# apple/ml-pgdvs

Measured on AMD Instinct MI355X. Metric: novel-view frames/s at 1080p x 24 src frames; achieved HBM GB/s vs gfx950 peak, higher is better.
Workload: dtype f32

## Files before the change

### ml-pgdvs_amd/csrc/knn_grid.hip

```cpp
#include <stdlib.h>

#include "common.h"
#include "fused.h"
#include "wave.h"

namespace pgdvs {

constexpr int kGridMaxCells = 1 << 24;
constexpr int kRingCap = 24;
constexpr int kRingCapAfterTpq = 3;
constexpr float kTargetPerCellDefault = 18.0f;

struct GridParams {
  float mn[3];
  float h, inv_h;
  int G[3];
  int ncells;
  int n;
  float sample_dist;
  int sample_dists;
};

__global__ void __launch_bounds__(256)
grid_bbox_kernel(const float *__restrict__ pts, const int32_t *__restrict__ count,
// ... 541 lines not shown
      *reinterpret_cast<int4 *>(out + idx) = q;
    } else if (idx <= n) {
      out[idx] = q.x;
      if (idx + 1 <= n) out[idx + 1] = q.y;
      if (idx + 2 <= n) out[idx + 2] = q.z;
    }
  }
  __syncthreads();
  }
}

__device__ __forceinline__ int wave_cell_take(int32_t *__restrict__ remaining, int c) {
  const int lane = threadIdx.x & 63;
  RunInfo r = wave_runs(c);
  int base = 0;
  if (r.is_leader && c >= 0) base = atomicSub(&remaining[c], r.length) - r.length;
  base = __shfl(base, r.leader, 64);
  return base + (lane - r.leader);
}

__global__ void __launch_bounds__(256)
grid_fill_kernel(const float *__restrict__ pts, const GridParams *__restrict__ gp,
                 const int32_t *__restrict__ cell_of, const int32_t *__restrict__ cell_start,
                 int32_t *__restrict__ cell_count, float4 *__restrict__ sorted,
                 const int32_t *__restrict__ gate) {
  if (gate && *gate == 0) return;
  const int n = gp->n;
  const int n_round = (n + 63) / 64 * 64;
  for (int i = blockIdx.x * blockDim.x + threadIdx.x; i < n_round; i += gridDim.x * blockDim.x) {
    const int c = i < n ? cell_of[i] : -1;
    const int slot = wave_cell_take(cell_count, c);
    if (i < n)
      sorted[cell_start[c] + slot] = make_float4(pts[(size_t)i * 3], pts[(size_t)i * 3 + 1], pts[(size_t)i * 3 + 2],
                                                 __int_as_float(i));
  }
}

struct BestList {
  float best;
  float mx;
};

__device__ __forceinline__ float readlane_f(float v, int l) {
  return __int_as_float(__builtin_amdgcn_readlane(__float_as_int(v), l));
}

__device__ __forceinline__ float wave_shift_up1_zero(float v) {
  int r = __builtin_amdgcn_update_dpp(0, __float_as_int(v), 0x138, 0xf, 0xf, true);
  return __int_as_float(r);
}

__device__ __forceinline__ void best_insert_batch(BestList &b, float d, bool valid, int KK, int lane) {
  (void)lane;
  unsigned long long mask = __ballot(valid && d < b.mx);
  if (!mask) return;
  while (mask) {
    int l = __builtin_ctzll(mask);
    mask &= mask - 1;
    float v = readlane_f(d, l);
    float up = wave_shift_up1_zero(b.best);
    b.best = __builtin_amdgcn_fmed3f(b.best, up, v);
  }
  b.mx = readlane_f(b.best, KK - 1);
}

template <int J>
__device__ __forceinline__ float lane_xor(float v, int lane) {
  const int iv = __float_as_int(v);
  if (J == 1) return __int_as_float(__builtin_amdgcn_update_dpp(iv, iv, 0xB1, 0xf, 0xf, false));
  if (J == 2) return __int_as_float(__builtin_amdgcn_update_dpp(iv, iv, 0x4E, 0xf, 0xf, false));
  if (J == 4) {
    int t = __builtin_amdgcn_update_dpp(iv, iv, 0x104, 0xf, 0x5, false);
    t = __builtin_amdgcn_update_dpp(t, iv, 0x114, 0xf, 0xa, false);
    return __int_as_float(t);
  }
  if (J == 8) return __int_as_float(__builtin_amdgcn_update_dpp(iv, iv, 0x128, 0xf, 0xf, false));
  if (J == 16) {
    auto r = __builtin_amdgcn_permlane16_swap(iv, iv, false, false);
    return __int_as_float((lane & 16) ? r[0] : r[1]);
  }
  auto r = __builtin_amdgcn_permlane32_swap(iv, iv, false, false);
  return __int_as_float((lane & 32) ? r[0] : r[1]);
}

template <int K, int J>
__device__ __forceinline__ float sort_step(float v, int lane) {
  const float o = lane_xor<J>(v, lane);
  const bool up = (lane & K) == 0;
  const bool lower = (lane & J) == 0;
  const float mn = fminf(v, o), mx = fmaxf(v, o);
  return (up == lower) ? mn : mx;
}

__device__ __forceinline__ float wave_sort_asc(float v, int lane) {
  v = sort_step<2, 1>(v, lane);
  v = sort_step<4, 2>(v, lane);
  v = sort_step<4, 1>(v, lane);
  v = sort_step<8, 4>(v, lane);
  v = sort_step<8, 2>(v, lane);
  v = sort_step<8, 1>(v, lane);
  v = sort_step<16, 8>(v, lane);
  v = sort_step<16, 4>(v, lane);
  v = sort_step<16, 2>(v, lane);
  v = sort_step<16, 1>(v, lane);
  v = sort_step<32, 16>(v, lane);
  v = sort_step<32, 8>(v, lane);
  v = sort_step<32, 4>(v, lane);
  v = sort_step<32, 2>(v, lane);
  v = sort_step<32, 1>(v, lane);
  v = sort_step<64, 32>(v, lane);
  v = sort_step<64, 16>(v, lane);
  v = sort_step<64, 8>(v, lane);
  v = sort_step<64, 4>(v, lane);
  v = sort_step<64, 2>(v, lane);
  v = sort_step<64, 1>(v, lane);
  return v;
}

__device__ __forceinline__ float dist2(float qx, float qy, float qz, float4 p) {
  float dx = qx - p.x, dy = qy - p.y, dz = qz - p.z;
  float d = dx * dx;
  d = d + dy * dy;
  d = d + dz * dz;
  return d;
}

__device__ __forceinline__ void scan_range(BestList &b, bool &first, const float4 *__restrict__ sorted,
                                           int start, int end, float qx, float qy, float qz, int KK,
                                           int lane, float bound = __builtin_inff()) {
  for (int j0 = start; j0 < end; j0 += 256) {
    float d[4];
    bool v[4];
#pragma unroll
    for (int u = 0; u < 4; ++u) {
      int j = j0 + u * 64 + lane;
      v[u] = j < end;
      float4 p = v[u] ? sorted[j] : make_float4(0.f, 0.f, 0.f, 0.f);
      d[u] = dist2(qx, qy, qz, p);
      v[u] = v[u] && d[u] <= bound;
    }
#pragma unroll
    for (int u = 0; u < 4; ++u) {
      if (j0 + u * 64 >= end) break;
      if (first) {
        b.best = wave_sort_asc(v[u] ? d[u] : __builtin_inff(), lane);
        b.mx = readlane_f(b.best, KK - 1);
        first = false;
      } else {
        best_insert_batch(b, d[u], v[u], KK, lane);
      }
    }
  }
}

struct QuerySrc {
  const float *qpts;
  const int32_t *qcount;
  int first_col;
  const int32_t *list;
  const int32_t *list_count;
  const float4 *qsorted;
};

__device__ __forceinline__ int query_count(const QuerySrc &qs, int n_points) {
  return qs.list ? *qs.list_count : (qs.qpts ? *qs.qcount : n_points);
}

__device__ __forceinline__ float4 load_query(const QuerySrc &qs, const float4 *__restrict__ sorted, int q) {
  if (qs.qpts == nullptr) return (qs.qsorted ? qs.qsorted : sorted)[q];
  return make_float4(qs.qpts[(size_t)q * 3], qs.qpts[(size_t)q * 3 + 1], qs.qpts[(size_t)q * 3 + 2],
                     __int_as_float(q));
}

__device__ __forceinline__ void knn_finish(float best, int KK, int first_col, int n, int lane, int orig,
                                           float *__restrict__ avg_out) {
  float s = (lane >= first_col && lane < KK && lane < n) ? best : 0.0f;
  s = wave_sum_down(s);
  if (lane == 0) avg_out[orig] = s / (float)(KK - first_col);
}

__device__ __forceinline__ float box_axis_dist2(float q, float mn, float h, int c0, int c1, int G) {
  float lo = c0 <= 0 ? -__builtin_inff() : mn + (float)c0 * h - 0.02f * h;
  float hi = c1 >= G - 1 ? __builtin_inff() : mn + (float)(c1 + 1) * h + 0.02f * h;
  float d = fmaxf(fmaxf(lo - q, q - hi), 0.0f);
  return d * d;
}

__device__ __forceinline__ void
grid_query_body(const GridParams *__restrict__ gp, const float4 *__restrict__ sorted,
                const CellIndex cell_start, int KK, QuerySrc qs, float *__restrict__ avg_out,
                int32_t *__restrict__ stats, int ring_cap, int32_t *__restrict__ fb_count,
                int32_t *__restrict__ fb_list, float *__restrict__ fb_bound) {
  const GridParams g = *gp;
  const int lane = threadIdx.x & 63;
  const int wave = __builtin_amdgcn_readfirstlane((int)(threadIdx.x >> 6));
  const int nq = query_count(qs, g.n);
  for (int qi = blockIdx.x * 4 + wave; qi < nq; qi += gridDim.x * 4) {
  const int q = qs.list ? qs.list[qi] : qi;
  const float4 qp = load_query(qs, sorted, q);
  const float qx = qp.x, qy = qp.y, qz = qp.z;
  const int orig = __float_as_int(qp.w);
  if (qs.qpts && !(isfinite(qx) && isfinite(qy) && isfinite(qz))) {
    if (lane == 0) avg_out[orig] = __builtin_nanf("");
    continue;
  }
  const int cx = cell_coord(qx, g.mn[0], g.inv_h, g.G[0]);
  const int cy = cell_coord(qy, g.mn[1], g.inv_h, g.G[1]);
  const int cz = cell_coord(qz, g.mn[2], g.inv_h, g.G[2]);
  BestList b;
  b.best = __builtin_inff();
  b.mx = __builtin_inff();
  bool first = true;
  bool done = false;
  int rings = 0;
  for (int r = 1; r <= ring_cap && !done; ++r) {
    rings = r;
    const int side = 2 * r + 1;
    const int nrows = side * side;
    for (int base = 0; base < nrows; base += 64) {
      int row_id = base + lane;
      if (r == 1) row_id = row_id < 9 ? (int)((0x862071534ull >> (row_id * 4)) & 15) : row_id;
      int s0 = 0, e0 = 0, s1 = 0, e1 = 0;
      float bd0 = 0.0f, bd1 = 0.0f;
      if (row_id < nrows) {
        int rz = (int)(((float)row_id + 0.5f) / (float)side);
        int dz = rz - r, dy = row_id - rz * side - r;
        int z = cz + dz, y = cy + dy;
        if (z >= 0 && z < g.G[2] && y >= 0 && y < g.G[1]) {
          int row = (z * g.G[1] + y) * g.G[0];
          float byz = box_axis_dist2(qy, g.mn[1], g.h, y, y, g.G[1]) + box_axis_dist2(qz, g.mn[2], g.h, z, z, g.G[2]);
          bool outer = r == 1 || dz == -r || dz == r || dy == -r || dy == r;
          if (outer) {
            int x0 = cx - r < 0 ? 0 : cx - r;
            int x1 = cx + r >= g.G[0] ? g.G[0] - 1 : cx + r;
            s0 = cell_start.at(row + x0);
            e0 = cell_start.at(row + x1 + 1);
            bd0 = byz + box_axis_dist2(qx, g.mn[0], g.h, x0, x1, g.G[0]);
          } else {
            if (cx - r >= 0) {
              s0 = cell_start.at(row + cx - r);
              e0 = cell_start.at(row + cx - r + 1);
              bd0 = byz + box_axis_dist2(qx, g.mn[0], g.h, cx - r, cx - r, g.G[0]);
            }
            if (cx + r < g.G[0]) {
              s1 = cell_start.at(row + cx + r);
              e1 = cell_start.at(row + cx + r + 1);
              bd1 = byz + box_axis_dist2(qx, g.mn[0], g.h, cx + r, cx + r, g.G[0]);
            }
          }
        }
      }
      unsigned long long m0 = __ballot(e0 > s0);
      while (m0) {
        int l = __builtin_ctzll(m0);
        m0 &= m0 - 1;
        if (readlane_f(bd0, l) >= b.mx) continue;
        scan_range(b, first, sorted, __builtin_amdgcn_readlane(s0, l), __builtin_amdgcn_readlane(e0, l), qx,
                   qy, qz, KK, lane);
      }
      unsigned long long m1 = __ballot(e1 > s1);
      while (m1) {
        int l = __builtin_ctzll(m1);
        m1 &= m1 - 1;
        if (readlane_f(bd1, l) >= b.mx) continue;
        scan_range(b, first, sorted, __builtin_amdgcn_readlane(s1, l), __builtin_amdgcn_readlane(e1, l), qx,
                   qy, qz, KK, lane);
      }
    }
    float db = __builtin_inff();
    bool open = false;
    const int c[3] = {cx, cy, cz};
    const float qv[3] = {qx, qy, qz};
#pragma unroll
    for (int a = 0; a < 3; ++a) {
      if (c[a] - r > 0) {
        open = true;
        db = fminf(db, qv[a] - (g.mn[a] + (float)(c[a] - r) * g.h));
      }
      if (c[a] + r < g.G[a] - 1) {
        open = true;
        db = fminf(db, (g.mn[a] + (float)(c[a] + r + 1) * g.h) - qv[a]);
      }
    }
    if (!open) {
      done = true;
    } else {
      float safe = db - 0.02f * g.h;
      if (safe > 0.0f && b.mx <= safe * safe) done = true;
    }
  }
  if (stats && lane == 0) atomicAdd(&stats[done ? (rings < 15 ? rings : 14) : 15], 1);
  if (!done) {
    if (lane == 0) {
      int slot = atomicAdd(fb_count, 1);
      fb_list[slot] = q;
      fb_bound[slot] = b.mx;
    }
    continue;
  }
  knn_finish(b.best, KK, qs.first_col, g.n, lane, orig, avg_out);
  }
}

constexpr int kTpqQueue = 8;
constexpr float kTpqRetryScale = 4.0f;

template <int KK>
__device__ __forceinline__ void tpq_insert(float (&a)[KK], float c) {
#pragma unroll
  for (int i = KK - 1; i > 0; --i) a[i] = __builtin_amdgcn_fmed3f(a[i - 1], a[i], c);
  asm("v_min_f32 %0, %1, %2" : "=v"(a[0]) : "v"(a[0]), "v"(c));
}

template <int KK>
__global__ void __launch_bounds__(256, 4)
grid_query_tpq_kernel(const GridParams *__restrict__ gp, const float4 *__restrict__ sorted,
                      const CellIndex cell_start, int first_col, float *__restrict__ avg_out,
                      int32_t *__restrict__ open_count, int32_t *__restrict__ open_list, float thr_mult) {
  __shared__ int2 s_run[9][256];
  __shared__ float s_bd[9][256];
  __shared__ float s_thr[256];
  __shared__ float s_safe[256];
  __shared__ unsigned long long s_order[256];
  const GridParams g = *gp;
  const int n = g.n;
  const int tid = threadIdx.x;
  for (int q0 = blockIdx.x * 256; q0 < n; q0 += gridDim.x * 256) {
  const int q = q0 + tid;
  const bool live = q < n;
  const float4 qp = sorted[live ? q : n - 1];
  const float qx = qp.x, qy = qp.y, qz = qp.z;
  float t0;
  {
  int ncand = 0;
  const int cx = cell_coord(qx, g.mn[0], g.inv_h, g.G[0]);
  const int cy = cell_coord(qy, g.mn[1], g.inv_h, g.G[1]);
  const int cz = cell_coord(qz, g.mn[2], g.inv_h, g.G[2]);
  const int x0 = cx - 1 < 0 ? 0 : cx - 1;
  const int x1 = cx + 1 >= g.G[0] ? g.G[0] - 1 : cx + 1;
#pragma unroll
  for (int k = 0; k < 9; ++k) {
    const int z = cz + k / 3 - 1, y = cy + k % 3 - 1;
    if (live && z >= 0 && z < g.G[2] && y >= 0 && y < g.G[1]) {
      const int row = (z * g.G[1] + y) * g.G[0];
      ncand += cell_start.at(row + x1 + 1) - cell_start.at(row + x0);
    }
  }
  t0 = (KK >= 17 && ncand >= KK) ? (KK >= 40 ? thr_mult : 6.0f) * (float)KK * g.h * g.h / (float)ncand : __builtin_inff();
  {
    float db = __builtin_inff();
    bool open = false;
    const int c[3] = {cx, cy, cz};
    const float qv[3] = {qx, qy, qz};
#pragma unroll
    for (int ax = 0; ax < 3; ++ax) {
      if (c[ax] - 1 > 0) {
        open = true;
        db = fminf(db, qv[ax] - (g.mn[ax] + (float)(c[ax] - 1) * g.h));
      }
      if (c[ax] + 1 < g.G[ax] - 1) {
        open = true;
        db = fminf(db, (g.mn[ax] + (float)(c[ax] + 2) * g.h) - qv[ax]);
      }
    }
    const float safe = db - 0.02f * g.h;
    s_safe[tid] = !open ? __builtin_inff() : (safe > 0.0f ? safe * safe : 0.0f);
  }
  }
  float a[KK];
  float mx;
  bool cut;
  for (int attempt = 0;; ++attempt) {
  {
  float lx = qx, ly = qy, lz = qz;
  asm volatile("" : "+v"(lx), "+v"(ly), "+v"(lz));
  const int cx = cell_coord(lx, g.mn[0], g.inv_h, g.G[0]);
  const int cy = cell_coord(ly, g.mn[1], g.inv_h, g.G[1]);
  const int cz = cell_coord(lz, g.mn[2], g.inv_h, g.G[2]);
  const int x0 = cx - 1 < 0 ? 0 : cx - 1;
  const int x1 = cx + 1 >= g.G[0] ? g.G[0] - 1 : cx + 1;
  const float bx = box_axis_dist2(lx, g.mn[0], g.h, x0, x1, g.G[0]);
  unsigned key[9];
#pragma unroll
  for (int k = 0; k < 9; ++k) {
    const int row_id = (int)((0x862071534ull >> (k * 4)) & 15);
    const int dz = row_id / 3 - 1, dy = row_id % 3 - 1;
    const int z = cz + dz, y = cy + dy;
    int2 se = make_int2(0, 0);
    float bd = 0.0f;
    if (live && z >= 0 && z < g.G[2] && y >= 0 && y < g.G[1]) {
      const int row = (z * g.G[1] + y) * g.G[0];
      const float byz = box_axis_dist2(ly, g.mn[1], g.h, y, y, g.G[1]) + box_axis_dist2(lz, g.mn[2], g.h, z, z, g.G[2]);
      bd = bx + byz;
      const float hw2 = t0 - byz;
      if (hw2 > 0.0f) {
        const float hw = __builtin_amdgcn_sqrtf(hw2) * 1.0001f + 0.02f * g.h;
        int f0 = fine_coord(lx - hw, g.mn[0], g.inv_h, g.G[0]);
        int f1 = fine_coord(lx + hw, g.mn[0], g.inv_h, g.G[0]);
        f0 = f0 < x0 * kSub ? x0 * kSub : f0;
        f1 = f1 > x1 * kSub + (kSub - 1) ? x1 * kSub + (kSub - 1) : f1;
        if (f0 <= f1) {
          se.x = cell_start.at_fine(row, f0);
          se.y = cell_start.at_fine(row, f1 + 1);
        }
      }
    }
    s_run[k][tid] = se;
    s_bd[k][tid] = bd;
    key[k] = se.y > se.x ? ((__float_as_uint(bd) & ~15u) | (unsigned)k) : (0xfffffff0u | (unsigned)k);
  }
  {
#define PGDVS_CE(i, j)                        \
  {                                           \
    const unsigned lo = key[i] < key[j] ? key[i] : key[j]; \
    key[j] = key[i] < key[j] ? key[j] : key[i];            \
    key[i] = lo;                              \
  }
    PGDVS_CE(0, 3) PGDVS_CE(1, 7) PGDVS_CE(2, 5) PGDVS_CE(4, 8)
    PGDVS_CE(0, 7) PGDVS_CE(2, 4) PGDVS_CE(3, 8) PGDVS_CE(5, 6)
    PGDVS_CE(0, 2) PGDVS_CE(1, 3) PGDVS_CE(4, 5) PGDVS_CE(7, 8)
    PGDVS_CE(1, 4) PGDVS_CE(3, 6) PGDVS_CE(5, 7)
    PGDVS_CE(0, 1) PGDVS_CE(2, 4) PGDVS_CE(3, 5) PGDVS_CE(6, 8)
    PGDVS_CE(2, 3) PGDVS_CE(4, 5) PGDVS_CE(6, 7)
    PGDVS_CE(1, 2) PGDVS_CE(3, 4) PGDVS_CE(5, 6)
#undef PGDVS_CE
  }
  {
    unsigned long long order = 0;
#pragma unroll
    for (int k = 0; k < 9; ++k) order |= (unsigned long long)(key[k] & 15u) << (4 * k);
    s_order[tid] = order;
  }
  }
  __builtin_amdgcn_sched_barrier(0);
  {
    s_thr[tid] = t0;
#pragma unroll
    for (int i = 0; i < KK; ++i) a[i] = t0;
  }
  mx = a[KK - 1];
  float qd[kTpqQueue];
#pragma unroll
  for (int u = 0; u < kTpqQueue; ++u) qd[u] = __builtin_inff();
  int qc = 0;
  int k = -1;
  unsigned j = 0u, e = 0u;
  auto push = [&](float d) {
#pragma unroll
    for (int u = kTpqQueue - 1; u > 0; --u) qd[u] = qd[u - 1];
    qd[0] = d;
    ++qc;
  };
  auto pop_insert = [&]() {
    tpq_insert<KK>(a, qd[0]);
#pragma unroll
    for (int u = 0; u + 1 < kTpqQueue; ++u) qd[u] = qd[u + 1];
    qd[kTpqQueue - 1] = __builtin_inff();
    qc = qc > 0 ? qc - 1 : 0;
    mx = a[KK - 1];
    __builtin_amdgcn_sched_barrier(0);
  };
  float4 ca0 = make_float4(0.f, 0.f, 0.f, 0.f), ca1 = ca0, cb0 = ca0, cb1 = ca0;
  bool va0 = false, va1 = false, vb0 = false, vb1 = false;
  auto step = [&](float4 &c_issue0, float4 &c_issue1, bool &v_issue0, bool &v_issue1, const float4 &c_use0,
                  const float4 &c_use1, const bool v_use0, const bool v_use1) -> bool {
    if (j >= e && k < 9) {
      ++k;
      if (k < 9) {
        const int row = (int)(s_order[tid] >> (4 * k)) & 15;
        const int2 se = s_run[row][tid];
        j = (unsigned)se.x * 16u;
        e = s_bd[row][tid] < mx ? (unsigned)se.y * 16u : j;
      }
    }
    v_issue0 = j < e;
    v_issue1 = j + 16u < e;
    c_issue0 = *reinterpret_cast<const float4 *>(reinterpret_cast<const char *>(sorted) + (size_t)(v_issue0 ? j : 0u));
    c_issue1 = *reinterpret_cast<const float4 *>(reinterpret_cast<const char *>(sorted) + (size_t)(v_issue1 ? j + 16u : 0u));
    j += (v_issue0 ? 16u : 0u) + (v_issue1 ? 16u : 0u);
    if (v_use0) {
      const float d = dist2(qx, qy, qz, c_use0);
      if (d < mx) push(d);
    }
    if (v_use1) {
      const float d = dist2(qx, qy, qz, c_use1);
      if (d < mx) push(d);
    }
    while (__builtin_amdgcn_ballot_w64(qc > kTpqQueue - 2) != 0) pop_insert();
    return __builtin_amdgcn_ballot_w64(v_issue0 || k < 9) != 0;
  };
  for (;;) {
    if (!step(cb0, cb1, vb0, vb1, ca0, ca1, va0, va1)) break;
    if (!step(ca0, ca1, va0, va1, cb0, cb1, vb0, vb1)) break;
  }
  while (__builtin_amdgcn_ballot_w64(qc > 0) != 0) pop_insert();
  mx = a[KK - 1];
  cut = mx < __builtin_inff() && mx == s_thr[tid];
  const float safe2 = s_safe[tid];
  const bool retry = cut && live && mx < safe2;
  if (attempt == 1 || __builtin_popcountll(__builtin_amdgcn_ballot_w64(retry)) < 16) break;
  t0 = retry ? fminf(kTpqRetryScale * t0, safe2) : t0;
  }
  if (!live) continue;
  const bool done = mx <= s_safe[tid];
  if (!done || cut || n < KK || first_col > 1) {
    open_list[atomicAdd(open_count, 1)] = q;
    continue;
  }
  a[0] = first_col == 1 ? 0.0f : a[0];
  int len = KK;
#pragma unroll
  for (int off = 32; off > 0; off >>= 1) {
#pragma unroll
    for (int i = 0; i < off; ++i)
      if (i + off < len) a[i] = a[i] + a[i + off];
    len = len < off ? len : off;
  }
  avg_out[__float_as_int(qp.w)] = a[0] / (float)(KK - first_col);
  }
}

__global__ void __launch_bounds__(256)
grid_query_kernel(const GridParams *__restrict__ gp, const float4 *__restrict__ sorted,
                  const CellIndex cell_start, int KK, QuerySrc qs, float *__restrict__ avg_out,
                  int32_t *__restrict__ stats, int ring_cap, int32_t *__restrict__ fb_count,
                  int32_t *__restrict__ fb_list, float *__restrict__ fb_bound) {
  grid_query_body(gp, sorted, cell_start, KK, qs, avg_out, stats, ring_cap, fb_count, fb_list, fb_bound);
}

__global__ void __launch_bounds__(256)
grid2_query_kernel(const GridParams *__restrict__ gp, const float4 *__restrict__ sorted,
                   const CellIndex cell_start, int KK, QuerySrc qs, float *__restrict__ avg_out,
                   int32_t *__restrict__ stats, int ring_cap, int32_t *__restrict__ fb_count,
                   int32_t *__restrict__ fb_list, float *__restrict__ fb_bound) {
  grid_query_body(gp, sorted, cell_start, KK, qs, avg_out, stats, ring_cap, fb_count, fb_list, fb_bound);
}

constexpr int kFbSlices = 16;
constexpr int kFbMaxSliced = 16384;

__global__ void __launch_bounds__(256)
grid_fallback_kernel(const GridParams *__restrict__ gp, const float4 *__restrict__ sorted, int KK,
                     QuerySrc qs, const int32_t *__restrict__ fb_count, const int32_t *__restrict__ fb_list,
                     const float *__restrict__ fb_bound, float *__restrict__ fb_partial) {
  __shared__ float s_best[4][64];
  const int n = gp->n;
  const int nfb = *fb_count;
  const int lane = threadIdx.x & 63;
  const int wave = __builtin_amdgcn_readfirstlane((int)(threadIdx.x >> 6));
  const int slice_len = ((n + kFbSlices - 1) / kFbSlices + 255) / 256 * 256;
  const int nsl = nfb < kFbMaxSliced ? nfb : kFbMaxSliced;
  for (int item = blockIdx.x; item < nsl * kFbSlices; item += gridDim.x) {
    const int f = item / kFbSlices, sl = item - f * kFbSlices;
    const float4 qp = load_query(qs, sorted, fb_list[f]);
    const float bound = fb_bound[f];
    BestList b;
    b.best = __builtin_inff();
    b.mx = __builtin_inff();
    bool first = true;
    const int s_beg = sl * slice_len;
    const int s_end = s_beg + slice_len < n ? s_beg + slice_len : n;
    for (int j0 = s_beg + wave * 256; j0 < s_end; j0 += 4 * 256) {
      int e = j0 + 256 < s_end ? j0 + 256 : s_end;
      scan_range(b, first, sorted, j0, e, qp.x, qp.y, qp.z, KK, lane, bound);
    }
    __syncthreads();
    s_best[wave][lane] = b.best;
    __syncthreads();
    if (wave == 0) {
      for (int w = 1; w < 4; ++w) best_insert_batch(b, s_best[w][lane], true, KK, lane);
      fb_partial[(size_t)item * 64 + lane] = b.best;
    }
  }
}

__global__ void __launch_bounds__(1024)
grid_fallback_finish_kernel(const GridParams *__restrict__ gp, const float4 *__restrict__ sorted, int KK,
                            QuerySrc qs, const int32_t *__restrict__ fb_count, const int32_t *__restrict__ fb_list,
                            const float *__restrict__ fb_bound, const float *__restrict__ fb_partial, float *__restrict__ avg_out,
                            const int32_t *__restrict__ scan_error) {
  __shared__ float s_best[16][64];
  const int n = gp->n;
  if (*scan_error != 0) {
    const int nq = query_count(qs, n);
    for (int i = blockIdx.x * blockDim.x + threadIdx.x; i < nq; i += gridDim.x * blockDim.x) avg_out[i] = __builtin_nanf("");
    return;
  }
  const int nfb = *fb_count;
  const int lane = threadIdx.x & 63;
  const int wave = __builtin_amdgcn_readfirstlane((int)(threadIdx.x >> 6));
  const int nsl = nfb < kFbMaxSliced ? nfb : kFbMaxSliced;
  for (int f = blockIdx.x * 16 + wave; f < nsl; f += gridDim.x * 16) {
    BestList b;
    b.best = fb_partial[((size_t)f * kFbSlices) * 64 + lane];
    b.mx = readlane_f(b.best, KK - 1);
    for (int sl = 1; sl < kFbSlices; ++sl)
      best_insert_batch(b, fb_partial[((size_t)f * kFbSlices + sl) * 64 + lane], true, KK, lane);
    knn_finish(b.best, KK, qs.first_col, n, lane, __float_as_int(load_query(qs, sorted, fb_list[f]).w), avg_out);
  }
  for (int f = kFbMaxSliced + blockIdx.x; f < nfb; f += gridDim.x) {
    const float4 qp = load_query(qs, sorted, fb_list[f]);
    const float bound = fb_bound[f];
    BestList b;
    b.best = __builtin_inff();
    b.mx = __builtin_inff();
    bool first = true;
    for (int j0 = wave * 256; j0 < n; j0 += 16 * 256) {
      int e = j0 + 256 < n ? j0 + 256 : n;
      scan_range(b, first, sorted, j0, e, qp.x, qp.y, qp.z, KK, lane, bound);
    }
    __syncthreads();
    s_best[wave][lane] = b.best;
    __syncthreads();
    if (wave == 0) {
      for (int w = 1; w < 16; ++w) best_insert_batch(b, s_best[w][lane], true, KK, lane);
      knn_finish(b.best, KK, qs.first_col, n, lane, __float_as_int(qp.w), avg_out);
    }
  }
}

struct GridWs {
  unsigned *bbox;
  GridParams *gp;
  int32_t *cell_of;
  float4 *samples;
  int32_t *sample_count;
  float *sample_d1;
  int sample_blocks;
  uint4 *tab;
  int32_t *occ_count, *occ_start, *nocc;
  float4 *sorted;
  int32_t *fb_count, *fb_list;
  int32_t *open_count, *open_list;
  float *fb_bound;
  float *fb_partial;
  unsigned long long *scan_state, *scan_state2, *rank_state;
  int32_t *scan_ticket, *scan_error;
  int scan_tiles;
  int64_t state_bytes;
  int32_t *stats;
  GridParams *gp2;
  int32_t *cell_count2, *cell_start2;
  float4 *sorted2;
  int32_t *fb2_count, *fb2_list;
  float *fb2_bound;
  int64_t total_bytes;
};

constexpr int kCoarseMaxCells = 1 << 18;
constexpr float kCoarseScale = 8.0f, kCoarseScaleMany = 4.0f;

static GridWs grid_ws_layout(void *base, int64_t capacity, int64_t qcapacity) {
  GridWs w;
  const int64_t points = capacity > 0 ? capacity : 1;
  const int64_t cells = points < kGridMaxCells ? points : (int64_t)kGridMaxCells;
  const int64_t occ_words = (cells + 2) * kSub;
  const int64_t queries = qcapacity > points ? qcapacity : points;
  Carver c{reinterpret_cast<char *>(base)};
  char *const state = c.take<char>(256);
  w.bbox = reinterpret_cast<unsigned *>(state);
  w.stats = reinterpret_cast<int32_t *>(state + 128);
  w.fb_count = reinterpret_cast<int32_t *>(state + 192);
  w.fb2_count = reinterpret_cast<int32_t *>(state + 196);
  w.open_count = reinterpret_cast<int32_t *>(state + 200);
  w.nocc = reinterpret_cast<int32_t *>(state + 204);
  w.scan_ticket = reinterpret_cast<int32_t *>(state + 216);
  w.scan_error = reinterpret_cast<int32_t *>(state + 224);
  w.scan_tiles = (int)(occ_words / kScanTile + 1);
  w.scan_state = c.take<unsigned long long>((int64_t)w.scan_tiles * 8, 8);
  w.scan_state2 = c.take<unsigned long long>((int64_t)(kCoarseMaxCells / kScanTile + 2) * 8, 8);
  w.rank_state = c.take<unsigned long long>((int64_t)(kRankBlocksMax + 1) * 8, 8);
  c.off = align_up(c.off, 256);
  w.state_bytes = c.off;
  w.gp = c.take<GridParams>(256);
  w.sample_blocks = (int)cdiv(points, kSampleBlock);
  w.samples = c.take<float4>((int64_t)w.sample_blocks * kSampleSlots * 16);
  w.sample_count = c.take<int32_t>((int64_t)w.sample_blocks * 4);
  w.sample_d1 = c.take<float>((int64_t)kSampleMaxQueries * 4);
  w.tab = c.take<uint4>((int64_t)kTabWords * 16);
  w.occ_count = c.take<int32_t>(occ_words * 4);
  w.occ_start = c.take<int32_t>(occ_words * 4);
  w.cell_of = c.take<int32_t>(points * 4);
  w.sorted = c.take<float4>(points * 16);
  w.fb_list = c.take<int32_t>(queries * 4);
  w.fb_bound = c.take<float>(queries * 4);
  w.open_list = c.take<int32_t>(points * 4);
  w.fb_partial = c.take<float>((int64_t)kFbMaxSliced * kFbSlices * 64 * 4);
  w.gp2 = c.take<GridParams>(256);
  w.cell_count2 = c.take<int32_t>(((int64_t)kCoarseMaxCells + 1) * 4);
  w.cell_start2 = c.take<int32_t>(((int64_t)kCoarseMaxCells + 1) * 4);
  w.sorted2 = c.take<float4>(points * 16);
  w.fb2_list = c.take<int32_t>(queries * 4);
  w.fb2_bound = c.take<float>(queries * 4);
  w.total_bytes = c.off;
  return w;
}

void knn_grid_counter_words(const void *workspace, int64_t capacity, int64_t qcapacity, const int32_t **to_ring,
                            const int32_t **to_coarse, const int32_t **to_exhaustive) {
  const GridWs w = grid_ws_layout(const_cast<void *>(workspace), capacity, qcapacity);
  *to_ring = w.open_count;
  *to_coarse = w.fb_count;
  *to_exhaustive = w.fb2_count;
}

int64_t knn_grid_workspace_bytes(int64_t capacity, int64_t qcapacity) {
  return grid_ws_layout(nullptr, capacity, qcapacity).total_bytes;
}

static int knn_grid_search(const float *pts, const int32_t *count, int64_t capacity, int K, float *avg_out,
                           void *workspace, int64_t workspace_bytes, hipStream_t st, const float *qpts,
                           const int32_t *qcount, int64_t qcapacity, bool prepared);

int knn_grid_mean_dist(const float *pts, const int32_t *count, int64_t capacity, int K, float *avg_out,
                       void *workspace, int64_t workspace_bytes, hipStream_t st, const float *qpts,
                       const int32_t *qcount, int64_t qcapacity) {
  return knn_grid_search(pts, count, capacity, K, avg_out, workspace, workspace_bytes, st, qpts, qcount, qcapacity, false);
}

void knn_grid_state_block(void *workspace, int64_t capacity, void **block, int64_t *bytes, unsigned **bbox, void **tab,
                          int64_t *tab_bytes, int32_t **occ_count, int *occ_mult, void **coarse, int64_t *coarse_bytes) {
  const GridWs ws = grid_ws_layout(workspace, capacity, 0);
  *block = ws.bbox;
  *bytes = ws.state_bytes;
  *bbox = ws.bbox;
  *tab = ws.tab;
  *tab_bytes = (int64_t)kTabWords * 16;
  *occ_count = ws.occ_count;
  *occ_mult = kSub;
  *coarse = ws.cell_count2;
  *coarse_bytes = align_up(((int64_t)kCoarseMaxCells + 1) * 4, 16);
}
int knn_grid_mean_dist_prepared(const float *pts, const int32_t *count, int64_t capacity, int K, float *avg_out, void *workspace,
                                int64_t workspace_bytes, hipStream_t st) {
  return knn_grid_search(pts, count, capacity, K, avg_out, workspace, workspace_bytes, st, nullptr, nullptr, 0, true);
}

static int knn_grid_search(const float *pts, const int32_t *count, int64_t capacity, int K, float *avg_out,
                           void *workspace, int64_t workspace_bytes, hipStream_t st, const float *qpts,
                           const int32_t *qcount, int64_t qcapacity, bool prepared) {
  GridWs ws = grid_ws_layout(workspace, capacity, qcapacity);
  const int KK = K + 1;
  QuerySrc qs;
  qs.qpts = qpts;
  qs.qcount = qcount;
  qs.first_col = qpts ? 0 : 1;
  qs.list = nullptr;
  qs.list_count = nullptr;
  qs.qsorted = nullptr;
  const int64_t nq_cap = qpts ? qcapacity : capacity;
  if (!workspace || workspace_bytes < ws.total_bytes) {
    set_error("knn_grid: workspace too small");
    return PGDVS_ERR_WORKSPACE;
  }
  unsigned gpts = (unsigned)(cdiv(capacity, 256) < 2048 ? cdiv(capacity, 256) : 2048);
  unsigned gbb = gpts < 128 ? gpts : 128;
  const float target = kTargetPerCellDefault * (float)(K + 1) / 51.0f;
  if (!prepared) {
    hipError_t e = hipMemsetAsync(ws.bbox, 0x00, (size_t)ws.state_bytes, st);
    if (e != hipSuccess) {
      set_error("knn_grid memset: %s", hipGetErrorString(e));
      return PGDVS_ERR_LAUNCH;
    }
    e = hipMemsetAsync(ws.cell_count2, 0x00, ((size_t)kCoarseMaxCells + 1) * 4, st);
    if (e != hipSuccess) {
      set_error("knn_grid memset: %s", hipGetErrorString(e));
      return PGDVS_ERR_LAUNCH;
    }
    PGDVS_LAUNCH("grid_bbox", grid_bbox_kernel, dim3(gbb), dim3(256), 0, st, pts, count, ws.bbox);
  }
  PGDVS_LAUNCH("grid_sample", grid_sample_kernel, dim3((unsigned)ws.sample_blocks), dim3(256), 0, st, pts, count, ws.samples,
               ws.sample_count);
  PGDVS_LAUNCH("grid_sample_nn", grid_sample_nn_kernel, dim3(kSampleMaxQueries), dim3(256), 0, st, count,
               (const float4 *)ws.samples, (const int32_t *)ws.sample_count, ws.sample_d1);
  PGDVS_LAUNCH("grid_params", grid_params_kernel, dim3(1), dim3(1024), 0, st, ws.bbox, count, (const float *)ws.sample_d1, ws.gp,
               sqrtf((float)(K + 1) / 51.0f), target, 0.5f);
  if (!prepared) PGDVS_LAUNCH("grid_tab_zero", grid_tab_zero_kernel, dim3(512), dim3(256), 0, st, ws.gp, ws.tab, ws.occ_count);
  PGDVS_LAUNCH("grid_mark", grid_mark_kernel, dim3(gpts), dim3(256), 0, st, pts, ws.gp, ws.cell_of, ws.tab);
  const unsigned nrb = (unsigned)cdiv(kTabWords, kRankWordsPerBlock);
  PGDVS_LAUNCH("grid_rank", grid_rank_kernel, dim3(nrb), dim3(1024), 0, st, ws.gp, ws.tab, ws.rank_state,
               reinterpret_cast<int32_t *>(ws.rank_state + kRankBlocksMax), ws.scan_error, ws.nocc);
  PGDVS_LAUNCH("grid_occ_count", grid_occ_count_kernel, dim3(gpts), dim3(256), 0, st, ws.gp, ws.cell_of,
               (const uint4 *)ws.tab, ws.occ_count);
  PGDVS_LAUNCH("grid_scan", grid_scan_kernel, dim3((unsigned)(ws.scan_tiles < kScanMaxBlocks ? ws.scan_tiles : kScanMaxBlocks)), dim3(1024), 0, st,
               ws.occ_count, (const int32_t *)(ws.nocc + 1), ws.occ_start, ws.scan_state, ws.scan_ticket, ws.scan_error);
  PGDVS_LAUNCH("grid_fill", grid_fill_kernel, dim3(gpts), dim3(256), 0, st, pts, ws.gp, ws.cell_of,
               ws.occ_start, ws.occ_count, ws.sorted, (const int32_t *)nullptr);
  CellIndex ci;
  ci.start = ws.occ_start;
  ci.tab = ws.tab;
  int32_t *const stats = option_int(options().knn_stats) != 0 ? ws.stats : nullptr;
  const unsigned gq = (unsigned)(cdiv(nq_cap, 4) < 256 * 8 ? (cdiv(nq_cap, 4) > 0 ? cdiv(nq_cap, 4) : 1) : 256 * 8);
  bool tpq = qpts == nullptr && option_int(options().knn_no_tpq) == 0 && capacity < (1ll << 27);
  const float thr_mult = 4.5f;
  if (tpq) {
    const unsigned gt = (unsigned)(cdiv(capacity, 256) < 2560 ? (cdiv(capacity, 256) > 0 ? cdiv(capacity, 256) : 1) : 2560);
    switch (KK) {
#define PGDVS_TPQ_CASE(N)                                                                                        \
  case N:                                                                                                        \
    PGDVS_LAUNCH("grid_query_tpq", grid_query_tpq_kernel<N>, dim3(gt), dim3(256), 0, st, ws.gp, ws.sorted,      \
// ... 61 lines not shown
```

Before: 1324.

## Move TPQ candidate queue to an LDS stack and store sorted cell keys

Measured after the change: 1340, median of 4. Within noise of the previous version (+1.2%).

```diff
diff --git a/ml-pgdvs_amd/csrc/knn_grid.hip b/ml-pgdvs_amd/csrc/knn_grid.hip
--- a/ml-pgdvs_amd/csrc/knn_grid.hip
+++ b/ml-pgdvs_amd/csrc/knn_grid.hip
@@ -867,7 +867,7 @@
   }
 }
 
-constexpr int kTpqQueue = 8;
+constexpr int kTpqQueue = 12;
 constexpr float kTpqRetryScale = 4.0f;
 
 template <int KK>
@@ -883,10 +883,10 @@
                       const CellIndex cell_start, int first_col, float *__restrict__ avg_out,
                       int32_t *__restrict__ open_count, int32_t *__restrict__ open_list, float thr_mult) {
   __shared__ int2 s_run[9][256];
-  __shared__ float s_bd[9][256];
-  __shared__ float s_thr[256];
+  __shared__ unsigned s_key[9][256];
+  __shared__ float s_tq[kTpqQueue][256];
+  static_assert(sizeof(int2) * 9 * 256 + 4 * 9 * 256 + 4 * kTpqQueue * 256 + 4 * 256 <= 163840 / 4, "LDS of four workgroups per CU");
   __shared__ float s_safe[256];
-  __shared__ unsigned long long s_order[256];
   const GridParams g = *gp;
   const int n = g.n;
   const int tid = threadIdx.x;
@@ -971,7 +971,6 @@
       }
     }
     s_run[k][tid] = se;
-    s_bd[k][tid] = bd;
     key[k] = se.y > se.x ? ((__float_as_uint(bd) & ~15u) | (unsigned)k) : (0xfffffff0u | (unsigned)k);
   }
   {
@@ -990,38 +989,32 @@
     PGDVS_CE(1, 2) PGDVS_CE(3, 4) PGDVS_CE(5, 6)
 #undef PGDVS_CE
   }
-  {
-    unsigned long long order = 0;
-#pragma unroll
-    for (int k = 0; k < 9; ++k) order |= (unsigned long long)(key[k] & 15u) << (4 * k);
-    s_order[tid] = order;
-  }
+#pragma unroll
+  for (int k = 0; k < 9; ++k) s_key[k][tid] = key[k];
   }
   __builtin_amdgcn_sched_barrier(0);
   {
-    s_thr[tid] = t0;
+    s_tq[0][tid] = t0;
 #pragma unroll
     for (int i = 0; i < KK; ++i) a[i] = t0;
   }
   mx = a[KK - 1];
-  float qd[kTpqQueue];
-#pragma unroll
-  for (int u = 0; u < kTpqQueue; ++u) qd[u] = __builtin_inff();
-  int qc = 0;
+  const int qa0 = tid * 4;
+  int qa = qa0;
+  float top = t0;
+  auto q_word = [&](int off) -> float & { return *reinterpret_cast<float *>(reinterpret_cast<char *>(&s_tq[0][0]) + off); };
   int k = -1;
   unsigned j = 0u, e = 0u;
   auto push = [&](float d) {
-#pragma unroll
-    for (int u = kTpqQueue - 1; u > 0; --u) qd[u] = qd[u - 1];
-    qd[0] = d;
-    ++qc;
+    q_word(qa) = top;
+    top = d;
+    qa += 1024;
   };
   auto pop_insert = [&]() {
-    tpq_insert<KK>(a, qd[0]);
-#pragma unroll
-    for (int u = 0; u + 1 < kTpqQueue; ++u) qd[u] = qd[u + 1];
-    qd[kTpqQueue - 1] = __builtin_inff();
-    qc = qc > 0 ? qc - 1 : 0;
+    qa = qa - 1024 > qa0 ? qa - 1024 : qa0;
+    const float below = q_word(qa);
+    tpq_insert<KK>(a, top);
+    top = below;
     mx = a[KK - 1];
     __builtin_amdgcn_sched_barrier(0);
   };
@@ -1032,10 +1025,10 @@
     if (j >= e && k < 9) {
       ++k;
       if (k < 9) {
-        const int row = (int)(s_order[tid] >> (4 * k)) & 15;
-        const int2 se = s_run[row][tid];
+        const unsigned key = s_key[k][tid];
+        const int2 se = s_run[key & 15u][tid];
         j = (unsigned)se.x * 16u;
-        e = s_bd[row][tid] < mx ? (unsigned)se.y * 16u : j;
+        e = __uint_as_float(key & ~15u) < mx ? (unsigned)se.y * 16u : j;
       }
     }
     v_issue0 = j < e;
@@ -1051,16 +1044,23 @@
       const float d = dist2(qx, qy, qz, c_use1);
       if (d < mx) push(d);
     }
-    while (__builtin_amdgcn_ballot_w64(qc > kTpqQueue - 2) != 0) pop_insert();
+    if (__builtin_amdgcn_ballot_w64(qa > qa0 + (kTpqQueue - 2) * 1024) != 0) {
+      pop_insert();
+      if (__builtin_amdgcn_ballot_w64(qa > qa0 + (kTpqQueue - 2) * 1024) != 0) pop_insert();
+    }
     return __builtin_amdgcn_ballot_w64(v_issue0 || k < 9) != 0;
   };
   for (;;) {
     if (!step(cb0, cb1, vb0, vb1, ca0, ca1, va0, va1)) break;
     if (!step(ca0, ca1, va0, va1, cb0, cb1, vb0, vb1)) break;
   }
-  while (__builtin_amdgcn_ballot_w64(qc > 0) != 0) pop_insert();
+#pragma unroll
+  for (int u = 0; u < kTpqQueue; ++u) {
+    if (__builtin_amdgcn_ballot_w64(qa > qa0) == 0) break;
+    pop_insert();
+  }
   mx = a[KK - 1];
-  cut = mx < __builtin_inff() && mx == s_thr[tid];
+  cut = mx < __builtin_inff() && mx == s_tq[0][tid];
   const float safe2 = s_safe[tid];
   const bool retry = cut && live && mx < safe2;
   if (attempt == 1 || __builtin_popcountll(__builtin_amdgcn_ballot_w64(retry)) < 16) break;
```
